# fdb/frequensea

Hardware: AMD Instinct MI355X
Metric: fft_frames_per_sec_n8192 (higher is better)
Workload: dtype f32

## Files before the change

### frequensea_amd/csrc/fsea_fft_core.h

```cpp
#pragma once

#include <hip/hip_runtime.h>
#include <stddef.h>
#include <stdint.h>

#include <fsea_pk_asm.h>
#include "fsea_opt.h"
#ifdef FSEA_TUNE
#include <fsea_pk_asm_tune.h>
#endif

namespace fsea {

constexpr int ilog2c(int n) {
    int l = 0;
    while ((1 << l) < n) ++l;
    return l;
}

constexpr int bitrev_c(int i, int bits) {
    int r = 0;
    for (int b = 0; b < bits; ++b) {
        if (i & (1 << b)) r |= 1 << (bits - 1 - b);
    }
    return r;
}

template <int P>
__host__ __device__ constexpr int lds_pad(int idx) {
    return idx + ((idx / P) << 1);
}

__host__ __device__ constexpr float cos64q(int i) {
    constexpr float t[17] = {1.000000000e+00f, 9.951847267e-01f, 9.807852804e-01f,
                             9.569403357e-01f, 9.238795325e-01f, 8.819212643e-01f,
                             8.314696123e-01f, 7.730104534e-01f, 7.071067812e-01f,
                             6.343932842e-01f, 5.555702330e-01f, 4.713967368e-01f,
                             3.826834324e-01f, 2.902846773e-01f, 1.950903220e-01f,
                             9.801714033e-02f, 0.0f};
    return t[i];
}
__host__ __device__ constexpr float cos64(int m) {
    m &= 63;
    if (m <= 16) return cos64q(m);
    if (m <= 32) return -cos64q(32 - m);
    if (m <= 48) return -cos64q(m - 32);
    return cos64q(64 - m);
}
__host__ __device__ constexpr float sin64(int m) { return cos64((m - 16) & 63); }

__device__ __forceinline__ cf cf_swap(cf b) { return __builtin_shufflevector(b, b, 1, 0); }
__device__ __forceinline__ cf cf_fma(cf a, cf b, cf c) { return __builtin_elementwise_fma(a, b, c); }

template <int L, int K>
__device__ __forceinline__ void bfly_const(cf &a, cf &b) {
    if constexpr (K == 0) {
        const cf t = b;
        b = a - t;
        a = a + t;
    } else if constexpr (4 * K == L) {
        const cf t = b;
        b = pk_add_pi(a, t);
        a = pk_add_mi(a, t);
    } else {
        constexpr int m = K * (64 / L);
        constexpr float wr = cos64(m), wi = -sin64(m);
        cf plus = cf_fma(b, cf{wr, wr}, a);
        plus = cf_fma(cf_swap(b), cf{-wi, wi}, plus);
        b = cf_fma(a, cf{2.0f, 2.0f}, -plus);
        a = plus;
    }
}

template <int R, int HALF, int BASE = 0, int K = 0>
__device__ __forceinline__ void dft_const_level(cf *y) {
    if constexpr (BASE < R) {
        bfly_const<2 * HALF, K>(y[BASE + K], y[BASE + K + HALF]);
        if constexpr (K + 1 < HALF) dft_const_level<R, HALF, BASE, K + 1>(y);
        else dft_const_level<R, HALF, BASE + 2 * HALF, 0>(y);
    }
}
template <int R, int HALF>
__device__ __forceinline__ void dft_const_levels(cf *y) {
    if constexpr (HALF < R) {
        dft_const_level<R, HALF>(y);
// ... 12 lines not shown
    dft_const_levels<R, 1>(y);
#pragma unroll
    for (int i = 0; i < R; ++i) x[i * S] = y[i];
}

template <int R, int S, int E0, int I = 0>
__device__ __forceinline__ void dft_win_level(const cf *x, const cf *wv, cf *y) {
    if constexpr (I < R / 2) {
        constexpr int BITS = ilog2c(R), EA = E0 + I * S, EB = E0 + (I + R / 2) * S;
        const cf a = x[I * S], b = x[(I + R / 2) * S];
        cf t;
        if constexpr (EB & 1) t = pk_scale_hi(b, wv[EB / 2]);
        else t = pk_scale_lo(b, wv[EB / 2]);
        if constexpr (EA & 1) {
            y[bitrev_c(I, BITS)] = pk_wfma_hi(a, wv[EA / 2], t);
            y[bitrev_c(I + R / 2, BITS)] = pk_wfms_hi(a, wv[EA / 2], t);
        } else {
            y[bitrev_c(I, BITS)] = pk_wfma_lo(a, wv[EA / 2], t);
            y[bitrev_c(I + R / 2, BITS)] = pk_wfms_lo(a, wv[EA / 2], t);
        }
        dft_win_level<R, S, E0, I + 1>(x, wv, y);
    }
}
template <int R, int S, int E0>
__device__ __forceinline__ void dft_regs_win(cf *x, const cf *wv) {
    static_assert(R >= 2 && R <= 64 && (R & (R - 1)) == 0, "radix must be 2..64");
    cf y[R];
    dft_win_level<R, S, E0>(x, wv, y);
    dft_const_levels<R, 2>(y);
#pragma unroll
    for (int i = 0; i < R; ++i) x[i * S] = y[i];
}

template <int R, int S, int TS>
__device__ __forceinline__ void dft_regs_tw(cf *x, const cf *tw, float sc0) {
    static_assert(R >= 4 && R <= 64 && (R & (R - 1)) == 0, "radix must be 4..64");
    constexpr int BITS = ilog2c(R);
    cf y[R];
#pragma unroll
    for (int i = 0; i < R / 2; ++i) {
        cf a = x[i * S];
        if (i == 0) {
            if (sc0 != 1.0f) a = a * cf{sc0, sc0};
        } else {
            a = pk_cmul(a, tw[(i - 1) * TS]);
        }
        const cf plus = pk_cmul_add(x[(i + R / 2) * S], tw[(i + R / 2 - 1) * TS], a);
        y[bitrev_c(i, BITS)] = plus;
        y[bitrev_c(i + R / 2, BITS)] = cf_fma(a, cf{2.0f, 2.0f}, -plus);
    }
    dft_const_levels<R, 2>(y);
#pragma unroll
    for (int i = 0; i < R; ++i) x[i * S] = y[i];
}

template <int R, int HALF, int TS, int DROP = 0>
__device__ __forceinline__ void dft_def_level(cf *y, const cf *tw) {
    if constexpr (HALF < R) {
        constexpr int OFF = HALF / 2, DISTINCT = HALF >= 2 ? HALF / 2 : 1;
#pragma unroll
        for (int base = 0; base < R; base += 2 * HALF) {
#pragma unroll
            for (int k = 0; k < DISTINCT; ++k) {
                cf &a = y[base + k], &b = y[base + k + HALF];
                const cf plus = pk_cmul_add(b, tw[(OFF + k) * TS], a);
                if constexpr (HALF <= DROP) b = a;
                else b = cf_fma(a, cf{2.0f, 2.0f}, -plus);
                a = plus;
            }
            if constexpr (HALF >= 2) {
#pragma unroll
                for (int k = 0; k < DISTINCT; ++k) {
                    cf &a = y[base + DISTINCT + k], &b = y[base + DISTINCT + k + HALF];
                    const cf plus = pk_cmul_add_mi(b, tw[(OFF + k) * TS], a);
                    if constexpr (HALF <= DROP) b = a;
                    else b = cf_fma(a, cf{2.0f, 2.0f}, -plus);
                    a = plus;
                }
            }
        }
        dft_def_level<R, 2 * HALF, TS, DROP>(y, tw);
    }
}

template <int R, int S, int TS, int DROP = 0>
__device__ __forceinline__ void dft_regs_def(cf *x, const cf *tw) {
    static_assert(R >= 4 && R <= 64 && (R & (R - 1)) == 0, "radix must be 4..64");
    constexpr int BITS = ilog2c(R);
    cf y[R];
#pragma unroll
    for (int i = 0; i < R; ++i) y[bitrev_c(i, BITS)] = x[i * S];
    dft_def_level<R, 1, TS, DROP>(y, tw);
#pragma unroll
    for (int i = 0; i < R; ++i) x[i * S] = y[i];
}

enum : int {
    MODE_MAG = 0,
    MODE_DB10_U8 = 1,
    MODE_DB5_U8_DCFIX = 2,
    MODE_COMPLEX = 3,
    MODE_MAG_NODC = 4,
    MODE_DB_F32 = 5
};
enum : int { IN_U8 = 0, IN_F32 = 1, IN_U8_ROT = 2 };

#ifndef FSEA_DEFAULT_OPT
#define FSEA_DEFAULT_OPT 0
#endif
#ifndef FSEA_STATIC_CONTIG
#define FSEA_STATIC_CONTIG 0
#endif
#ifndef FSEA_TRACE
#define FSEA_TRACE 0
#endif

template <int N_, int T_, int FPW_, int WPE_, int NP_, int R0_, int R1_, int R2_ = 1, int R3_ = 1,
          bool TWL_ = true, bool TWR_ = true, int ABL_ = 0, int OPT_ = FSEA_DEFAULT_OPT>
struct FftCfg {
    static constexpr int OPT = OPT_;
    static constexpr int ABL = ABL_;
    static constexpr int N = N_, T = T_, FPW = FPW_, NP = NP_;
    static constexpr int WPE = WPE_;
    static constexpr int P = N_ / T_;
    static constexpr int WG = T_ * FPW_;
// ... 40 lines not shown
    const float *win = nullptr;
    const cf *win_dc = nullptr;
    uint32_t win_offset = 0;
};

template <int C>
__device__ __forceinline__ void ld_c(const cf *p, cf *dst) {
    if constexpr (C == 1) {
        dst[0] = *p;
    } else {
#pragma unroll
        for (int c = 0; c < C; c += 2) {
            const cf2 q = *reinterpret_cast<const cf2 *>(p + c);
            dst[c] = cf{q[0], q[1]};
            dst[c + 1] = cf{q[2], q[3]};
        }
    }
}

template <int C>
__device__ __forceinline__ void st_c(cf *p, const cf *src) {
    if constexpr (C == 1) {
        *p = src[0];
    } else {
#pragma unroll
        for (int c = 0; c < C; c += 2) {
            *reinterpret_cast<cf2 *>(p + c) = cf2{src[c][0], src[c][1], src[c + 1][0], src[c + 1][1]};
        }
    }
}

typedef __amdgpu_buffer_rsrc_t rsrc_t;

__device__ __forceinline__ rsrc_t buffer_window(const void *base, size_t off, size_t total) {
    const size_t rem = total > off ? total - off : 0;
    char *p = const_cast<char *>(static_cast<const char *>(base)) + (rem ? off : 0);
    return __builtin_amdgcn_make_buffer_rsrc(p, 0, rem > 0xffffffffull ? 0xffffffffu : (uint32_t)rem, 0x00020000);
}

typedef uint32_t u32x2 __attribute__((vector_size(8)));
typedef uint32_t u32x4 __attribute__((vector_size(16)));

__device__ __forceinline__ uint32_t f2u(float x) { return __builtin_bit_cast(uint32_t, x); }
__device__ __forceinline__ float u2f(uint32_t x) { return __builtin_bit_cast(float, x); }

#ifndef FSEA_STORE_GUARD
#define FSEA_STORE_GUARD 1
#endif
__device__ __forceinline__ void store_data_guard() {
#if !defined(__AMDGCN__)
#elif FSEA_STORE_GUARD == 1
    __builtin_amdgcn_sched_barrier(0);
    asm volatile("s_nop 7\n\ts_nop 7");
    __builtin_amdgcn_sched_barrier(0);
#elif FSEA_STORE_GUARD >= 10
    __builtin_amdgcn_sched_barrier(0);
    asm volatile("s_nop %0" ::"n"(FSEA_STORE_GUARD - 10));
    __builtin_amdgcn_sched_barrier(0);
#endif
}

template <int AUX>
__device__ __forceinline__ void bst128(rsrc_t rs, uint32_t voff, uint32_t soff, u32x4 data) {
#if FSEA_STORE_GUARD == 2
    __builtin_amdgcn_raw_buffer_store_b64(u32x2{data[0], data[1]}, rs, voff, soff, AUX);
    __builtin_amdgcn_raw_buffer_store_b64(u32x2{data[2], data[3]}, rs, voff + 8, soff, AUX);
#else
    __builtin_amdgcn_raw_buffer_store_b128(data, rs, voff, soff, AUX);
    store_data_guard();
#endif
// ... 99 lines not shown
    double s, c;
    sincospi(2.0 * turns, &s, &c);
    return cf{(float)c, (float)s};
}
__device__ __forceinline__ cf turn_phasor_f32(double turns) {
    turns -= floor(turns);
    float s, c;
    sincospif(2.0f * (float)turns, &s, &c);
    return cf{c, s};
}

template <class Cfg, int IN, int MODE_T = -1, bool ROT = false, bool RUNS = false, int WIN = 0>
struct FftKernel {
    static_assert(!ROT || IN == IN_U8, "the fused frequency shift is a u8-input path");
    static_assert(WIN == 0 || (Cfg::TWR && (Cfg::OPT & opt::TUNE_ONLY) == 0 && Cfg::P >= 8),
                  "the windowed kernels: V1 schedule, register-resident last-pass twiddles");
    static_assert(WIN == 0 || !RUNS || (IN == IN_U8 && !ROT), "windowed half-overlap runs: the plain u8 kernel only");
    static constexpr bool WIN_DC = WIN != 0 && IN == IN_U8;
    static constexpr bool LATE_LOAD = WIN != 0 && IN == IN_F32;
    static constexpr bool DC_IN_REGS = WIN_DC && ((Cfg::OPT & opt::WIN_DC_REGS) != 0 ||
                                                  ((Cfg::OPT & opt::WIN_DC_REGS_MAG) != 0 && MODE_T == MODE_MAG && !ROT));
    static_assert(!RUNS || (IN == IN_U8 && !ROT && Cfg::FPW == 1 && (Cfg::R(0) % 2) == 0), "half-overlap runs: u8 input, one frame per workgroup");
    static constexpr int N = Cfg::N, T = Cfg::T, P = Cfg::P, NP = Cfg::NP, FPW = Cfg::FPW;
    static constexpr int LAST = NP - 1;
    static constexpr int R0 = Cfg::R(0), C0 = Cfg::C(0);
    static constexpr int RL = Cfg::R(LAST), CL = Cfg::C(LAST), NsL = Cfg::Ns(LAST);
    static constexpr bool ONE_WAVE = (Cfg::WG <= 64) || (T <= 64 && (64 % T) == 0);
    static constexpr float SC = (IN == IN_U8) ? (1.0f / 256.0f) : 1.0f;
    static constexpr bool PRESCALED = Cfg::TWR && (IN == IN_U8);
    using Raw = RawRow<IN, C0>;
    static constexpr bool BATCH_READS = (Cfg::OPT & opt::BATCH_READS) != 0;
    static constexpr bool TW_HOIST = (Cfg::OPT & opt::TW_HOIST) != 0;
    static constexpr bool TW_FUSE = (Cfg::OPT & opt::TW_FUSE) != 0 && (Cfg::ABL & abl::NO_FLOPS) == 0;
    static constexpr int ST_AUX = (Cfg::OPT & opt::ST_NT) ? 2 : 0;
    template <int ELEM_BYTES>
    static constexpr int st_aux() { return (T * CL * ELEM_BYTES >= 128 && CL * ELEM_BYTES <= 16) ? ST_AUX : (ST_AUX & ~2); }
    static constexpr int LD_AUX = (Cfg::OPT & opt::LD_NT) ? 2 : 0;
    static constexpr bool DEFER = (Cfg::OPT & opt::DEFER) != 0 && NP == 3;
    static constexpr bool PX_PACK = (Cfg::OPT & opt::PX_PACK) != 0;
    static constexpr bool PX_BIAS = (Cfg::OPT & opt::PX_BIAS) != 0;
    static constexpr bool LANE_ROT = (Cfg::OPT & opt::LANE_ROT) != 0;
    static constexpr bool LANE_ROT_LAST = (Cfg::OPT & opt::LANE_ROT_LAST) != 0;
    template <int I>
    static __device__ __forceinline__ int pass_lane(int t) {
        constexpr bool ON = (I == LAST) ? LANE_ROT_LAST : LANE_ROT;
        if constexpr (ON && Cfg::C(I) == 2 && P == 32 && (T % 16) == 0) {
            const int blk = t >> 4;
            return (blk << 4) | ((t - blk) & 15);
        } else if constexpr (ON && Cfg::C(I) == 1 && P == 16 && T == 256) {
            const int blk = t >> 4;
            const int logical = (blk >> 1) | ((blk & 1) << 3);
            return (logical << 4) | (t & 15);
        } else {
            return t;
        }
    }

    static __device__ __forceinline__ void after_reads() {
        if constexpr (BATCH_READS) __builtin_amdgcn_sched_barrier(0);
    }

    static __device__ __forceinline__ void frame_sync() {
        if constexpr (Cfg::ABL & abl::NO_LDS) {
            return;
        } else if constexpr (ONE_WAVE) {
            __builtin_amdgcn_fence(__ATOMIC_RELEASE, "wavefront");
// ... 105 lines not shown
                for (int r = 0; r < R; ++r) lds[Cfg::pad(j0 + r * Ns)] = v[r * C + c];
            }
        }
    }

    template <int I>
    static __device__ __forceinline__ void lds_read(const cf *lds, cf *v, int t) {
        constexpr int R = Cfg::R(I), C = Cfg::C(I);
        constexpr int STRIDE = N / R;
        if constexpr (Cfg::ABL & abl::NO_LDS) {
            return;
        } else if constexpr (STRIDE % P == 0) {
            const cf *base = lds + Cfg::pad(C * t);
#pragma unroll
            for (int r = 0; r < R; ++r) ld_c<C>(base + r * (STRIDE + 2 * (STRIDE / P)), v + r * C);
        } else {
#pragma unroll
            for (int r = 0; r < R; ++r) ld_c<C>(lds + Cfg::pad(C * t + r * STRIDE), v + r * C);
        }
    }

    template <int I>
    static __device__ __forceinline__ void middle_pass(cf *lds, const cf *lds_all, cf *v, const FftArgs &a, int t0,
                                                       const cf *tw_res = nullptr) {
        if constexpr (I < LAST) {
            constexpr int R = Cfg::R(I), C = Cfg::C(I);
            const int t = pass_lane<I>(t0);
            const cf *tw = Cfg::TWL ? (lds_all + Cfg::lds_tw_off(I)) : a.tw[I];
            if constexpr (DEFER) {
                lds_read<I>(lds, v, t);
                after_reads();
                frame_sync();
#pragma unroll
                for (int c = 0; c < C; ++c) dft_regs_def<R, C, 1, (Cfg::ABL & abl::DROP_32_OPS) ? 2 : ((Cfg::ABL & abl::DROP_16_OPS) ? 1 : 0)>(v + c, tw_res + c * (R / 2));
            } else if constexpr (TW_HOIST && (Cfg::Ns(I) % C == 0)) {
                constexpr int Ns = Cfg::Ns(I);
                cf w[(R - 1) * C];
                const int k0 = (C * t) % Ns;
#pragma unroll
                for (int r = 1; r < R; ++r) ld_c<C>(tw + (r - 1) * Ns + k0, w + (r - 1) * C);
                lds_read<I>(lds, v, t);
                after_reads();
                frame_sync();
                if constexpr (TW_FUSE) {
#pragma unroll
                    for (int c = 0; c < C; ++c) dft_regs_tw<R, C, C>(v + c, w + c, 1.0f);
                } else {
#pragma unroll
                    for (int r = 1; r < R; ++r) {
#pragma unroll
                        for (int c = 0; c < C; ++c) v[r * C + c] = pk_cmul(v[r * C + c], w[(r - 1) * C + c]);
                    }
                }
            } else {
                lds_read<I>(lds, v, t);
                after_reads();
                frame_sync();
                apply_twiddles<I>(v, tw, t);
            }
            if constexpr (!DEFER && !(TW_FUSE && TW_HOIST && (Cfg::Ns(I) % C == 0))) {
#pragma unroll
                for (int c = 0; c < C; ++c) dft_regs<R, C, (Cfg::ABL & abl::NO_FLOPS) != 0>(v + c);
            }
            lds_write<I>(lds, v, t);
            frame_sync();
            middle_pass<I + 1>(lds, lds_all, v, a, t0, tw_res);
        }
    }

    static __device__ __forceinline__ uint32_t elem_bytes(int mode) {
        return (mode == MODE_DB10_U8 || mode == MODE_DB5_U8_DCFIX) ? 1u : (mode == MODE_COMPLEX ? 8u : 4u);
    }

    static __device__ __forceinline__ float bin_power(const cf *v, int r, int c) {
        const cf z = v[r * CL + c];
        return __builtin_fmaf(z[0], z[0], z[1] * z[1]);
    }

    static __device__ __forceinline__ void epilogue(int mode, rsrc_t out, uint32_t lane_elem, cf *v, int t) {
        constexpr float SE = PRESCALED ? 1.0f : SC;
        constexpr float SE2 = SE * SE;
        const bool patched = (mode == MODE_MAG) || (mode == MODE_DB5_U8_DCFIX);
        if (WIN == 0 && IN == IN_U8 && !patched && t == 0) {
            const float dc = (PRESCALED ? 0.5f : 128.0f) * (float)N;
            v[(RL / 2) * CL] += cf{dc, dc};
        }
        if (mode == MODE_COMPLEX) {
            const uint32_t voff = lane_elem * 8u;
#pragma unroll
            for (int r = 0; r < RL; ++r) {
                cf z[CL];
#pragma unroll
                for (int c = 0; c < CL; ++c) z[c] = v[r * CL + c] * cf{SE, SE};
                bst<CL, st_aux<8>()>(out, voff, (uint32_t)(r * NsL) * 8u, z);
            }
        } else if (mode == MODE_DB10_U8 || mode == MODE_DB5_U8_DCFIX) {
            const float kdb = (mode == MODE_DB10_U8 ? 100.0f : 50.0f) * 0.30102999566398120f;
            const uint32_t voff = lane_elem;
#pragma unroll
            for (int r = 0; r < RL; ++r) {
                const uint32_t soff = (uint32_t)(r * NsL);
                uint8_t px[CL];
                [[maybe_unused]] uint32_t pxw[(CL + 3) / 4] = {};
#pragma unroll
                for (int c = 0; c < CL; ++c) {
                    float p = bin_power(v, r, c);
                    if constexpr (!PRESCALED && IN == IN_U8) p *= SE2;
                    if constexpr (PX_PACK) {
                        float d;
                        if constexpr (PX_BIAS) d = __builtin_fmaf(kdb, __builtin_amdgcn_logf(p), -0.49999997f);
                        else d = trunc_f32(kdb * __builtin_amdgcn_logf(p));
                        if constexpr (Cfg::ABL & abl::NO_EPILOGUE_MATH) d = kdb * p;
                        pxw[c / 4] = cvt_pk_u8(d, (uint32_t)(c & 3), pxw[c / 4]);
                    } else {
                        float d = kdb * __builtin_amdgcn_logf(p);
                        if constexpr (Cfg::ABL & abl::NO_EPILOGUE_MATH) d = kdb * p;
                        int q = (int)d;
                        q = q < 0 ? 0 : (q > 255 ? 255 : q);
                        px[c] = (uint8_t)q;
                    }
                }
                if constexpr (PX_PACK) {
#pragma unroll
                    for (int c = 0; c < CL; ++c) px[c] = (uint8_t)(pxw[c / 4] >> (8 * (c & 3)));
                }
                if constexpr (Cfg::ABL & abl::NO_STORES) {
                    if (px[0] == 255 && px[CL - 1] == 254 && v[0][0] == -1.0f) bst<CL>(out, voff, soff, px);
                } else if (patched && r == RL / 2 && t == 0) {
#pragma unroll
                    for (int c = 1; c < CL; ++c) bst<1>(out, voff + c, soff, px + c);
                } else if constexpr (PX_PACK) {
                    if constexpr (CL == 1) __builtin_amdgcn_raw_buffer_store_b8((uint8_t)pxw[0], out, voff, soff, st_aux<1>());
                    else if constexpr (CL == 2) __builtin_amdgcn_raw_buffer_store_b16((uint16_t)pxw[0], out, voff, soff, st_aux<1>());
                    else {
#pragma unroll
                        for (int c = 0; c < CL; c += 4) __builtin_amdgcn_raw_buffer_store_b32(pxw[c / 4], out, voff + c, soff, st_aux<1>());
                    }
                } else {
                    bst<CL, st_aux<1>()>(out, voff, soff, px);
                }
                if (patched && r == RL / 2 - 1 && t == T - 1) bst<1>(out, voff + CL, soff, px + (CL - 1));
            }
        } else if (mode == MODE_DB_F32) {
            f32_rows<true>(patched, out, lane_elem, v, t);
        } else {
            f32_rows<false>(patched, out, lane_elem, v, t);
        }
    }

    template <bool LOG>
    static __device__ __forceinline__ void f32_rows(bool patched, rsrc_t out, uint32_t lane_elem, cf *v, int t) {
        constexpr float SE = PRESCALED ? 1.0f : SC;
        constexpr float SE2 = SE * SE;
        const uint32_t voff = lane_elem * 4u;
#pragma unroll
        for (int r = 0; r < RL; ++r) {
            const uint32_t soff = (uint32_t)(r * NsL) * 4u;
            float m[CL];
#pragma unroll
            for (int c = 0; c < CL; ++c) {
                float p = bin_power(v, r, c);
                if constexpr (!PRESCALED && IN == IN_U8) p *= SE2;
                if constexpr (LOG) {
                    m[c] = (10.0f * 0.30102999566398120f) * __builtin_amdgcn_logf(p + 1.0e-20f);
                } else if constexpr (Cfg::ABL & abl::NO_EPILOGUE_MATH) {
                    m[c] = v[r * CL + c][0];
                } else {
                    m[c] = __builtin_amdgcn_sqrtf(p);
                }
            }
            if constexpr (Cfg::ABL & abl::NO_STORES) {
                if (m[0] == -1.0f) bst<CL>(out, voff, soff, m);
            } else if (patched && r == RL / 2 && t == 0) {
#pragma unroll
                for (int c = 1; c < CL; ++c) bst<1>(out, voff + 4 * c, soff, m + c);
                if constexpr (CL >= 4) store_data_guard();
            } else {
                bst<CL, st_aux<4>()>(out, voff, soff, m);
            }
            if (patched && r == RL / 2 - 1 && t == T - 1) bst<1>(out, voff + 4 * CL, soff, m + (CL - 1));
        }
    }

    static constexpr bool DYNAMIC = !ONE_WAVE;
    static constexpr unsigned POOLS = 8;
    static constexpr unsigned NO_UNIT = 0xffffffffu;

    struct Pools {
        unsigned n_units, grid;
        __device__ __forceinline__ unsigned start(unsigned q) const { return (unsigned)((size_t)n_units * q / POOLS); }
        __device__ __forceinline__ unsigned homed(unsigned q) const { return (grid + POOLS - 1 - q) / POOLS; }
        __device__ __forceinline__ unsigned unit(unsigned q, unsigned t) const {
            const unsigned long long idx = (unsigned long long)start(q) + homed(q) + t;
            return idx < start(q + 1) ? (unsigned)idx : NO_UNIT;
        }
    };

#ifdef FSEA_TUNE
    static constexpr bool V2 = (Cfg::OPT & opt::V2) != 0, W64 = (Cfg::OPT & opt::W64) != 0;
#else
    static constexpr bool V2 = false, W64 = false;
    static_assert((Cfg::OPT & opt::TUNE_ONLY) == 0 && Cfg::ABL == 0, "tuning-only option or ablation in a product build");
#endif
    static constexpr int counters_used() { return W64 ? 0 : (V2 ? 2 : (DYNAMIC ? 1 : 0)); }

    static constexpr int WPAIRS = WIN ? P / 2 : 1;
    static constexpr int DC_OFF = (Cfg::LDS_ALLOC + 1) & ~1;
    static constexpr int LDS_CF = (WIN_DC && !DC_IN_REGS) ? DC_OFF + 2 * NsL : Cfg::LDS_ALLOC;
    static constexpr int DC_REGS = (2 * NsL + Cfg::WG - 1) / Cfg::WG;
    static_assert(WIN == 0 || (Cfg::TWL || Cfg::TWR), "the DC table rides on the table block's barrier");
    static __device__ __forceinline__ void load_window(rsrc_t rs, int t, cf *wv) {
        const uint32_t voff = (uint32_t)t * 16u;
#pragma unroll
// ... 42 lines not shown

    static __device__ __forceinline__ void run_v1(const FftArgs &a, cf *lds_all) {
        const int tid = threadIdx.x;
        const int slot = (FPW == 1) ? 0 : tid / T;
        const int t = (FPW == 1) ? tid : tid % T;
        cf *lds = lds_all + slot * Cfg::LDS_FRAME;
        unsigned *tk = reinterpret_cast<unsigned *>(lds_all + Cfg::LDS_TOTAL);

        const unsigned b = blockIdx.x;
        const bool issuer = (tid == 0);
        const size_t n_units = RUNS ? (a.n_frames + a.run_len - 1) / a.run_len : (a.n_frames + FPW - 1) / FPW;
        Pools pools;
        pools.n_units = (unsigned)n_units;
        pools.grid = gridDim.x;
        unsigned cur = b % POOLS;

        if ((FSEA_TRACE != 0) && a.trace != nullptr && tid == 0) {
            const unsigned hw_id = read_hw_id(), xcc_id = read_xcc_id();
            a.trace[32 * b + 0] = wall_clock64();
            a.trace[32 * b + 2] = __builtin_readcyclecounter();
            a.trace[32 * b + 4] = hw_id;
            a.trace[32 * b + 5] = xcc_id;
        }

        const int mode = (MODE_T >= 0) ? MODE_T : a.mode;
        const uint32_t xormask = (MODE_T >= 0) ? 0u : a.xormask;
        const uint32_t esz = elem_bytes(mode);
        const size_t total_in = (size_t)IN_BPS * ((a.n_frames - 1) * a.hop + (size_t)N);
        const bool tiled = a.tile_rows != 0;
        const size_t total_out = (size_t)esz * (tiled ? a.out_span : a.n_frames * (size_t)N);
        const uint32_t in_voff = (uint32_t)IN_BPS * ((uint32_t)slot * (uint32_t)a.hop + (uint32_t)(C0 * t));
        const int tl = pass_lane<LAST>(t);
        const uint32_t out_elem = (uint32_t)slot * (tiled ? a.pitch_row : (uint32_t)N) + (uint32_t)(CL * tl);
        auto row_elem = [&](size_t f) -> size_t {
            if (!tiled) return f * (size_t)N;
            const uint32_t k = (uint32_t)f / a.tile_rows, y = (uint32_t)f - k * a.tile_rows;
            return (size_t)y * a.pitch_row + (size_t)k * a.pitch_tile;
        };

        size_t u = b;
#if FSEA_STATIC_CONTIG
        [[maybe_unused]] const size_t contig_per = (n_units + gridDim.x - 1) / gridDim.x;
        [[maybe_unused]] size_t contig_end = n_units;
        if constexpr (!RUNS) {
            u = (size_t)b * contig_per;
            contig_end = u + contig_per < n_units ? u + contig_per : n_units;
            if (u >= n_units) u = n_units;
        }
#endif
        unsigned tick_next = 0;
        const bool dyn = !RUNS && DYNAMIC && a.dynamic_units != 0;
        [[maybe_unused]] size_t fcur = RUNS ? (size_t)b * a.run_len : 0;
        [[maybe_unused]] unsigned jpos = 0;
        if (dyn) {
            u = (size_t)pools.start(cur) + b / POOLS;
            if (u >= pools.start(cur + 1)) u = n_units;
        }
        constexpr int TAB_COPY = (Cfg::TWL || Cfg::TWR) ? Cfg::TAB_SMALL : 0;
        constexpr int TAB_REGS = (TAB_COPY + Cfg::WG - 1) / Cfg::WG;
        cf tabv[TAB_REGS > 0 ? TAB_REGS : 1];
#pragma unroll
        for (int i = 0; i < TAB_REGS; ++i) {
            const int e = tid + i * Cfg::WG;
            tabv[i] = a.tw_small[e < TAB_COPY ? e : TAB_COPY - 1];
        }
        constexpr int R1 = Cfg::R(1), C1 = Cfg::C(1), Ns1 = Cfg::Ns(1);
        cf tw1[DEFER ? C1 * (R1 / 2) : 1];
        if constexpr (DEFER) {
            const int t1 = pass_lane<1>(t);
#pragma unroll
            for (int c = 0; c < C1; ++c) ld_c<R1 / 2>(a.tw_def + ((C1 * t1 + c) % Ns1) * (R1 / 2), tw1 + c * (R1 / 2));
        }
        [[maybe_unused]] const rsrc_t win_rs = buffer_window(WIN ? a.win : nullptr, 0, WIN ? (size_t)N * 4u : 0);
        cf wv[WPAIRS];
        cf dcv[(WIN_DC && !DC_IN_REGS) ? DC_REGS : 1];
        cf dcr[DC_IN_REGS ? 2 * CL : 1];
        if constexpr (DC_IN_REGS) {
#pragma unroll
            for (int c = 0; c < CL; ++c) {
                dcr[c] = a.win_dc[CL * tl + c];
                dcr[CL + c] = a.win_dc[NsL + CL * tl + c];
            }
        }
        if constexpr (WIN != 0) load_window(win_rs, t, wv);
        if constexpr (WIN_DC && !DC_IN_REGS) {
#pragma unroll
            for (int i = 0; i < DC_REGS; ++i) {
                const int e = tid + i * Cfg::WG;
                dcv[i] = a.win_dc[e < 2 * NsL ? e : 2 * NsL - 1];
            }
        }
        if (dyn) {
            if (issuer) tick_next = atomicAdd(a.ctr + 32 * cur, 1u);
        }
        Raw raw[R0];
        load_raw(buffer_window(a.in, (size_t)IN_BPS * (RUNS ? fcur : u * FPW) * a.hop, u < n_units ? total_in : 0), in_voff, raw);
        balance_vmcnt();

        if constexpr (TAB_COPY > 0) {
#pragma unroll
            for (int i = 0; i < TAB_REGS; ++i) {
                const int e = tid + i * Cfg::WG;
                lds_all[FPW * Cfg::LDS_FRAME + (e < TAB_COPY ? e : TAB_COPY - 1)] = tabv[i];
            }
            if constexpr (WIN_DC && !DC_IN_REGS) {
#pragma unroll
                for (int i = 0; i < DC_REGS; ++i) {
                    const int e = tid + i * Cfg::WG;
                    lds_all[DC_OFF + (e < 2 * NsL ? e : 2 * NsL - 1)] = dcv[i];
                }
            }
            if ((FSEA_TRACE != 0) && a.trace != nullptr && tid == 0) a.trace[32 * b + 28] = wall_clock64();
            __syncthreads();
            if ((FSEA_TRACE != 0) && a.trace != nullptr && tid == 0) a.trace[32 * b + 29] = wall_clock64();
        }
        cf twl[Cfg::TWR ? (RL - 1) * CL : 1];
        if constexpr (Cfg::TWR) {
            const cf *hi = lds_all + Cfg::LDS_HI, *lo = lds_all + Cfg::LDS_LO;
            auto root = [&](unsigned m) -> cf { return pk_cmul(hi[m >> 6], lo[m & 63u]); };
            constexpr int RB = RL >= 16 ? 8 : (RL >= 4 ? 2 : RL);
            constexpr int RA = RL / RB;
#pragma unroll
            for (int c = 0; c < CL; ++c) {
                const unsigned k = (unsigned)(CL * tl + c);
                cf wb[RB], wa[RA];
#pragma unroll
                for (int bb = 1; bb < RB; ++bb) wb[bb] = root((unsigned)bb * k);
#pragma unroll
                for (int aa = 1; aa < RA; ++aa) wa[aa] = root((unsigned)(RB * aa) * k);
#pragma unroll
                for (int r = 1; r < RL; ++r) {
                    const int aa = r / RB, bb = r % RB;
                    cf w = aa == 0 ? wb[bb] : (bb == 0 ? wa[aa] : pk_cmul(wa[aa], wb[bb]));
                    if constexpr (PRESCALED) w = w * cf{SC, SC};
                    twl[(r - 1) * CL + c] = w;
                }
            }
        }

        cf ebase[ROT ? C0 : 1];
        if constexpr (ROT) {
#pragma unroll
            for (int c = 0; c < C0; ++c) {
                const unsigned n0 = (unsigned)(C0 * t + c);
                const cf e = turn_phasor_f64(a.rot_delta * (double)n0);
                ebase[c] = (WIN == 0 && (n0 & 1u)) ? -e : e;
            }
        }

        unsigned par = 0;
        if (dyn && u >= n_units) {
            if (issuer) {
                unsigned nu = pools.unit(cur, tick_next);
                for (unsigned k = 1; nu == NO_UNIT && k < POOLS; ++k) {
                    const unsigned q = (cur + k) % POOLS;
                    nu = pools.unit(q, atomicAdd(a.ctr + 32 * q, 1u));
                    if (nu != NO_UNIT) cur = q;
                }
                tk[0] = nu;
                tick_next = atomicAdd(a.ctr + 32 * cur, 1u);
            }
            __syncthreads();
            const unsigned nu = __builtin_amdgcn_readfirstlane(tk[0]);
            __syncthreads();
            u = (nu == NO_UNIT) ? n_units : (size_t)nu;
            load_raw(buffer_window(a.in, (size_t)IN_BPS * (u * FPW) * a.hop, u < n_units ? total_in : 0), in_voff, raw);
            balance_vmcnt();
        }

        unsigned iter = 0;
        if ((FSEA_TRACE != 0) && a.trace != nullptr && tid == 0) a.trace[32 * b + 6] = wall_clock64();
        while (u < n_units) {
            if (dyn && issuer) {
                unsigned nu = pools.unit(cur, tick_next);
                for (unsigned k = 1; nu == NO_UNIT && k < POOLS; ++k) {
                    const unsigned q = (cur + k) % POOLS;
                    nu = pools.unit(q, atomicAdd(a.ctr + 32 * q, 1u));
                    if (nu != NO_UNIT) cur = q;
                }
                tk[par] = nu;
                tick_next = atomicAdd(a.ctr + 32 * cur, 1u);
            }

            cf v[P];
            if constexpr (ROT) {
                const size_t first = (u * FPW + (size_t)slot) * a.hop;
                const cf ef = turn_phasor_f32(a.rot_phase0 + a.rot_delta * (double)first);
                cf fr[C0];
#pragma unroll
                for (int c = 0; c < C0; ++c) fr[c] = pk_cmul(ebase[c], ef);
#pragma unroll
                for (int r = 0; r < R0; ++r) {
                    convert_row<IN, C0, false>(raw[r], a.xormask, C0 * t, v + r * C0);
                    const cf wr = a.rot_row[r];
#pragma unroll
                    for (int c = 0; c < C0; ++c) {
                        v[r * C0 + c] = pk_cmul(v[r * C0 + c] + cf{128.0f, 128.0f}, pk_cmul_uniform(fr[c], wr));
                        if constexpr (WIN != 0) {
                            if (a.win_offset != 0) v[r * C0 + c] += cf{128.0f, 128.0f};
                        }
                    }
                }
            } else if constexpr (WIN != 0 && IN == IN_F32) {
#pragma unroll
                for (int r = 0; r < R0; ++r) convert_row<IN, C0, false>(raw[r], 0u, C0 * t, v + r * C0);
// ... 5 lines not shown
                for (int r = 0; r < R0; ++r) convert_row<IN, C0>(raw[r], xormask, C0 * t, v + r * C0);
            }
            if ((FSEA_TRACE != 0) && a.trace != nullptr && tid == 0 && iter == 0) {
                asm volatile("" ::"v"(v[0]));
                a.trace[32 * b + 30] = wall_clock64();
            }
            if constexpr (WIN != 0) {
                pass0_windowed(v, wv);
            } else {
#pragma unroll
                for (int c = 0; c < C0; ++c) dft_regs<R0, C0, (Cfg::ABL & abl::NO_FLOPS) != 0>(v + c);
            }
            lds_write<0>(lds, v, t);
            frame_sync();
            if ((FSEA_TRACE != 0) && a.trace != nullptr && tid == 0 && iter == 0) a.trace[32 * b + 7] = wall_clock64();
            size_t un = u + gridDim.x;
#if FSEA_STATIC_CONTIG
            if constexpr (!RUNS) un = u + 1 < contig_end ? u + 1 : n_units;
#endif
            [[maybe_unused]] size_t fnext = 0;
            [[maybe_unused]] bool same_run = false;
            if constexpr (RUNS) {
                same_run = (jpos + 1 < a.run_len) && (fcur + 1 < a.n_frames);
                un = same_run ? u : u + gridDim.x;
                fnext = same_run ? fcur + 1 : un * (size_t)a.run_len;
            }
            if (dyn) {
                if constexpr (Cfg::ABL & abl::NO_LDS) __syncthreads();
                const unsigned nu = __builtin_amdgcn_readfirstlane(tk[par]);
                par ^= 1u;
                un = (nu == NO_UNIT) ? n_units : (size_t)nu;
            }
            if constexpr (RUNS) {
                const rsrc_t rs = buffer_window(a.in, (size_t)IN_BPS * fnext * a.hop, un < n_units ? total_in : 0);
                if (same_run) {
#pragma unroll
                    for (int r = 0; r < R0 / 2; ++r) raw[r] = raw[r + R0 / 2];
                    load_raw_rows<R0 / 2, R0>(rs, in_voff, raw);
                } else {
                    load_raw(rs, in_voff, raw);
                }
            } else if constexpr ((Cfg::ABL & abl::NO_LOADS) == 0 && !LATE_LOAD) {
                load_raw(buffer_window(a.in, (size_t)IN_BPS * (un * FPW) * a.hop, un < n_units ? total_in : 0), in_voff, raw);
            }
            middle_pass<1>(lds, lds_all, v, a, t, tw1);

            lds_read<LAST>(lds, v, tl);
            after_reads();
            frame_sync();
            if constexpr (Cfg::TWR && TW_FUSE) {
#pragma unroll
                for (int c = 0; c < CL; ++c) dft_regs_tw<RL, CL, CL>(v + c, twl + c, PRESCALED ? SC : 1.0f);
            } else if constexpr (Cfg::TWR) {
                if constexpr (PRESCALED) {
#pragma unroll
                    for (int c = 0; c < CL; ++c) v[c] = v[c] * cf{SC, SC};
                }
#pragma unroll
                for (int r = 1; r < RL; ++r) {
#pragma unroll
                    for (int c = 0; c < CL; ++c) {
                        if constexpr (Cfg::ABL & abl::NO_FLOPS) v[r * CL + c] += twl[(r - 1) * CL + c];
                        else v[r * CL + c] = pk_cmul(v[r * CL + c], twl[(r - 1) * CL + c]);
                    }
                }
            } else {
                apply_twiddles<LAST>(v, a.tw[LAST], tl);
            }
            if constexpr (!(Cfg::TWR && TW_FUSE)) {
#pragma unroll
                for (int c = 0; c < CL; ++c) dft_regs<RL, CL, (Cfg::ABL & abl::NO_FLOPS) != 0>(v + c);
            }
            if constexpr (DC_IN_REGS) {
#pragma unroll
                for (int c = 0; c < CL; ++c) {
                    v[(RL / 2 - 1) * CL + c] += dcr[c];
                    v[(RL / 2) * CL + c] += dcr[CL + c];
                }
            }
            if constexpr (WIN_DC && !DC_IN_REGS) {
                constexpr int CB = CL >= 2 ? 2 : 1;
#pragma unroll
                for (int c = 0; c < CL; c += CB) {
                    cf dc_lo[CB], dc_hi[CB];
                    ld_c<CB>(lds_all + DC_OFF + CL * tl + c, dc_lo);
                    ld_c<CB>(lds_all + DC_OFF + NsL + CL * tl + c, dc_hi);
#pragma unroll
                    for (int j = 0; j < CB; ++j) {
                        v[(RL / 2 - 1) * CL + c + j] += dc_lo[j];
                        v[(RL / 2) * CL + c + j] += dc_hi[j];
                    }
                }
            }
            if constexpr (WIN != 0) {
                if constexpr (WIN == 1) {
                    load_window(win_rs, t, wv);
                    __builtin_amdgcn_sched_barrier(0);
                }
            }
            epilogue(mode, buffer_window(a.out, (size_t)esz * row_elem(RUNS ? fcur : u * FPW), total_out), out_elem, v, tl);
            if constexpr (LATE_LOAD) {
                load_raw(buffer_window(a.in, (size_t)IN_BPS * (un * FPW) * a.hop, un < n_units ? total_in : 0), in_voff, raw);
            }
            u = un;
            if constexpr (RUNS) {
                fcur = fnext;
                jpos = same_run ? jpos + 1 : 0;
            }
            if ((FSEA_TRACE != 0) && a.trace != nullptr && tid == 0 && iter < 24) a.trace[32 * b + 8 + iter] = wall_clock64();
            ++iter;
        }

        if (dyn && issuer) {
            __builtin_amdgcn_s_waitcnt(0);
            const unsigned finished = atomicAdd(a.ctr + 32 * POOLS, 1u);
            if (finished == gridDim.x - 1) {
#pragma unroll
                for (unsigned q = 0; q <= POOLS; ++q) a.ctr[32 * q] = 0;
            }
        }
        if ((FSEA_TRACE != 0) && a.trace != nullptr && tid == 0) {
            a.trace[32 * b + 1] = wall_clock64();
            a.trace[32 * b + 3] = __builtin_readcyclecounter();
        }
    }
};

}
```

Measured before the change: 86.33 million.

## Fuse twiddle butterflies into packed-FMA asm and force scalar unit-window math

Adds inline-asm packed FMA sequences that compute the twiddled butterfly (plus and minus outputs) in three v_pk_fma instructions, used in the register DFT passes for the plain u8 input kernel. It also moves the buffer-window and unit-bound computations onto scalar registers via readfirstlane so the 64-bit comparisons are not done per lane. Lane-flag checks in the epilogue are forced into VGPRs to steer codegen. The aim is fewer VALU instructions and less vector register pressure, at the risk of the hand-written asm defeating compiler scheduling or carrying op_sel mistakes.

```diff
diff --git a/frequensea_amd/csrc/fsea_fft_core.h b/frequensea_amd/csrc/fsea_fft_core.h
--- a/frequensea_amd/csrc/fsea_fft_core.h
+++ b/frequensea_amd/csrc/fsea_fft_core.h
@@ -6,6 +6,7 @@
 
 #include <fsea_pk_asm.h>
 #include "fsea_opt.h"
+#include "fsea_unit_window.h"
 #ifdef FSEA_TUNE
 #include <fsea_pk_asm_tune.h>
 #endif
@@ -51,6 +52,10 @@
 
 __device__ __forceinline__ cf cf_swap(cf b) { return __builtin_shufflevector(b, b, 1, 0); }
 __device__ __forceinline__ cf cf_fma(cf a, cf b, cf c) { return __builtin_elementwise_fma(a, b, c); }
+
+}
+#include "fsea_pk_fused.h"
+namespace fsea {
 
 template <int L, int K>
 __device__ __forceinline__ void bfly_const(cf &a, cf &b) {
@@ -129,7 +134,7 @@
     for (int i = 0; i < R; ++i) x[i * S] = y[i];
 }
 
-template <int R, int S, int TS>
+template <int R, int S, int TS, bool FUSED = false>
 __device__ __forceinline__ void dft_regs_tw(cf *x, const cf *tw, float sc0) {
     static_assert(R >= 4 && R <= 64 && (R & (R - 1)) == 0, "radix must be 4..64");
     constexpr int BITS = ilog2c(R);
@@ -139,19 +144,27 @@
         cf a = x[i * S];
         if (i == 0) {
             if (sc0 != 1.0f) a = a * cf{sc0, sc0};
+        } else if constexpr (FUSED) {
+            a = pk_cmul_fused(a, tw[(i - 1) * TS]);
         } else {
             a = pk_cmul(a, tw[(i - 1) * TS]);
         }
-        const cf plus = pk_cmul_add(x[(i + R / 2) * S], tw[(i + R / 2 - 1) * TS], a);
-        y[bitrev_c(i, BITS)] = plus;
-        y[bitrev_c(i + R / 2, BITS)] = cf_fma(a, cf{2.0f, 2.0f}, -plus);
+        if constexpr (FUSED) {
+            cf b = x[(i + R / 2) * S];
+            y[bitrev_c(i, BITS)] = pk_bfly_cmul(a, b, tw[(i + R / 2 - 1) * TS]);
+            y[bitrev_c(i + R / 2, BITS)] = b;
+        } else {
+            const cf plus = pk_cmul_add(x[(i + R / 2) * S], tw[(i + R / 2 - 1) * TS], a);
+            y[bitrev_c(i, BITS)] = plus;
+            y[bitrev_c(i + R / 2, BITS)] = cf_fma(a, cf{2.0f, 2.0f}, -plus);
+        }
     }
     dft_const_levels<R, 2>(y);
 #pragma unroll
     for (int i = 0; i < R; ++i) x[i * S] = y[i];
 }
 
-template <int R, int HALF, int TS, int DROP = 0>
+template <int R, int HALF, int TS, int DROP = 0, bool FUSED = false>
 __device__ __forceinline__ void dft_def_level(cf *y, const cf *tw) {
     if constexpr (HALF < R) {
         constexpr int OFF = HALF / 2, DISTINCT = HALF >= 2 ? HALF / 2 : 1;
@@ -160,34 +173,42 @@
 #pragma unroll
             for (int k = 0; k < DISTINCT; ++k) {
                 cf &a = y[base + k], &b = y[base + k + HALF];
-                const cf plus = pk_cmul_add(b, tw[(OFF + k) * TS], a);
-                if constexpr (HALF <= DROP) b = a;
-                else b = cf_fma(a, cf{2.0f, 2.0f}, -plus);
-                a = plus;
-            }
-            if constexpr (HALF >= 2) {
-#pragma unroll
-                for (int k = 0; k < DISTINCT; ++k) {
-                    cf &a = y[base + DISTINCT + k], &b = y[base + DISTINCT + k + HALF];
-                    const cf plus = pk_cmul_add_mi(b, tw[(OFF + k) * TS], a);
+                if constexpr (FUSED && HALF > DROP) {
+                    a = pk_bfly_cmul(a, b, tw[(OFF + k) * TS]);
+                } else {
+                    const cf plus = pk_cmul_add(b, tw[(OFF + k) * TS], a);
                     if constexpr (HALF <= DROP) b = a;
                     else b = cf_fma(a, cf{2.0f, 2.0f}, -plus);
                     a = plus;
                 }
             }
-        }
-        dft_def_level<R, 2 * HALF, TS, DROP>(y, tw);
-    }
-}
-
-template <int R, int S, int TS, int DROP = 0>
+            if constexpr (HALF >= 2) {
+#pragma unroll
+                for (int k = 0; k < DISTINCT; ++k) {
+                    cf &a = y[base + DISTINCT + k], &b = y[base + DISTINCT + k + HALF];
+                    if constexpr (FUSED && HALF > DROP) {
+                        a = pk_bfly_cmul_mi(a, b, tw[(OFF + k) * TS]);
+                    } else {
+                        const cf plus = pk_cmul_add_mi(b, tw[(OFF + k) * TS], a);
+                        if constexpr (HALF <= DROP) b = a;
+                        else b = cf_fma(a, cf{2.0f, 2.0f}, -plus);
+                        a = plus;
+                    }
+                }
+            }
+        }
+        dft_def_level<R, 2 * HALF, TS, DROP, FUSED>(y, tw);
+    }
+}
+
+template <int R, int S, int TS, int DROP = 0, bool FUSED = false>
 __device__ __forceinline__ void dft_regs_def(cf *x, const cf *tw) {
     static_assert(R >= 4 && R <= 64 && (R & (R - 1)) == 0, "radix must be 4..64");
     constexpr int BITS = ilog2c(R);
     cf y[R];
 #pragma unroll
     for (int i = 0; i < R; ++i) y[bitrev_c(i, BITS)] = x[i * S];
-    dft_def_level<R, 1, TS, DROP>(y, tw);
+    dft_def_level<R, 1, TS, DROP, FUSED>(y, tw);
 #pragma unroll
     for (int i = 0; i < R; ++i) x[i * S] = y[i];
 }
@@ -294,10 +315,17 @@
 
 typedef __amdgpu_buffer_rsrc_t rsrc_t;
 
+template <bool SCALAR = false>
 __device__ __forceinline__ rsrc_t buffer_window(const void *base, size_t off, size_t total) {
-    const size_t rem = total > off ? total - off : 0;
-    char *p = const_cast<char *>(static_cast<const char *>(base)) + (rem ? off : 0);
-    return __builtin_amdgcn_make_buffer_rsrc(p, 0, rem > 0xffffffffull ? 0xffffffffu : (uint32_t)rem, 0x00020000);
+    if constexpr (SCALAR) {
+        const ByteWindow w = byte_window(off, total);
+        char *p = const_cast<char *>(static_cast<const char *>(base)) + w.base_off;
+        return __builtin_amdgcn_make_buffer_rsrc(p, 0, w.num_records, 0x00020000);
+    } else {
+        const size_t rem = total > off ? total - off : 0;
+        char *p = const_cast<char *>(static_cast<const char *>(base)) + (rem ? off : 0);
+        return __builtin_amdgcn_make_buffer_rsrc(p, 0, rem > 0xffffffffull ? 0xffffffffu : (uint32_t)rem, 0x00020000);
+    }
 }
 
 typedef uint32_t u32x2 __attribute__((vector_size(8)));
@@ -463,6 +491,8 @@
     static constexpr bool BATCH_READS = (Cfg::OPT & opt::BATCH_READS) != 0;
     static constexpr bool TW_HOIST = (Cfg::OPT & opt::TW_HOIST) != 0;
     static constexpr bool TW_FUSE = (Cfg::OPT & opt::TW_FUSE) != 0 && (Cfg::ABL & abl::NO_FLOPS) == 0;
+    static constexpr bool PK_FUSED = WIN == 0 && IN == IN_U8 && !ROT;
+    static constexpr bool SCALAR_UNITS = PK_FUSED;
     static constexpr int ST_AUX = (Cfg::OPT & opt::ST_NT) ? 2 : 0;
     template <int ELEM_BYTES>
     static constexpr int st_aux() { return (T * CL * ELEM_BYTES >= 128 && CL * ELEM_BYTES <= 16) ? ST_AUX : (ST_AUX & ~2); }
@@ -634,7 +664,7 @@
                 after_reads();
                 frame_sync();
 #pragma unroll
-                for (int c = 0; c < C; ++c) dft_regs_def<R, C, 1, (Cfg::ABL & abl::DROP_32_OPS) ? 2 : ((Cfg::ABL & abl::DROP_16_OPS) ? 1 : 0)>(v + c, tw_res + c * (R / 2));
+                for (int c = 0; c < C; ++c) dft_regs_def<R, C, 1, (Cfg::ABL & abl::DROP_32_OPS) ? 2 : ((Cfg::ABL & abl::DROP_16_OPS) ? 1 : 0), PK_FUSED>(v + c, tw_res + c * (R / 2));
             } else if constexpr (TW_HOIST && (Cfg::Ns(I) % C == 0)) {
                 constexpr int Ns = Cfg::Ns(I);
                 cf w[(R - 1) * C];
@@ -646,7 +676,7 @@
                 frame_sync();
                 if constexpr (TW_FUSE) {
 #pragma unroll
-                    for (int c = 0; c < C; ++c) dft_regs_tw<R, C, C>(v + c, w + c, 1.0f);
+                    for (int c = 0; c < C; ++c) dft_regs_tw<R, C, C, PK_FUSED>(v + c, w + c, 1.0f);
                 } else {
 #pragma unroll
                     for (int r = 1; r < R; ++r) {
@@ -677,6 +707,17 @@
     static __device__ __forceinline__ float bin_power(const cf *v, int r, int c) {
         const cf z = v[r * CL + c];
         return __builtin_fmaf(z[0], z[0], z[1] * z[1]);
+    }
+
+    static __device__ __forceinline__ bool lane_flag(bool f) {
+#if defined(__AMDGCN__)
+        if constexpr (PK_FUSED && MODE_T >= 0 && CL <= 2) {
+            uint32_t x = f ? 1u : 0u;
+            asm("" : "+v"(x));
+            return x != 0;
+        }
+#endif
+        return f;
     }
 
     static __device__ __forceinline__ void epilogue(int mode, rsrc_t out, uint32_t lane_elem, cf *v, int t) {
@@ -699,6 +740,7 @@
         } else if (mode == MODE_DB10_U8 || mode == MODE_DB5_U8_DCFIX) {
             const float kdb = (mode == MODE_DB10_U8 ? 100.0f : 50.0f) * 0.30102999566398120f;
             const uint32_t voff = lane_elem;
+            const bool first_lane = lane_flag(t == 0), last_lane = lane_flag(t == T - 1);
 #pragma unroll
             for (int r = 0; r < RL; ++r) {
                 const uint32_t soff = (uint32_t)(r * NsL);
@@ -728,7 +770,7 @@
                 }
                 if constexpr (Cfg::ABL & abl::NO_STORES) {
                     if (px[0] == 255 && px[CL - 1] == 254 && v[0][0] == -1.0f) bst<CL>(out, voff, soff, px);
-                } else if (patched && r == RL / 2 && t == 0) {
+                } else if (patched && r == RL / 2 && first_lane) {
 #pragma unroll
                     for (int c = 1; c < CL; ++c) bst<1>(out, voff + c, soff, px + c);
                 } else if constexpr (PX_PACK) {
@@ -741,7 +783,7 @@
                 } else {
                     bst<CL, st_aux<1>()>(out, voff, soff, px);
                 }
-                if (patched && r == RL / 2 - 1 && t == T - 1) bst<1>(out, voff + CL, soff, px + (CL - 1));
+                if (patched && r == RL / 2 - 1 && last_lane) bst<1>(out, voff + CL, soff, px + (CL - 1));
             }
         } else if (mode == MODE_DB_F32) {
             f32_rows<true>(patched, out, lane_elem, v, t);
@@ -755,6 +797,7 @@
         constexpr float SE = PRESCALED ? 1.0f : SC;
         constexpr float SE2 = SE * SE;
         const uint32_t voff = lane_elem * 4u;
+        const bool first_lane = lane_flag(t == 0), last_lane = lane_flag(t == T - 1);
 #pragma unroll
         for (int r = 0; r < RL; ++r) {
             const uint32_t soff = (uint32_t)(r * NsL) * 4u;
@@ -773,14 +816,14 @@
             }
             if constexpr (Cfg::ABL & abl::NO_STORES) {
                 if (m[0] == -1.0f) bst<CL>(out, voff, soff, m);
-            } else if (patched && r == RL / 2 && t == 0) {
+            } else if (patched && r == RL / 2 && first_lane) {
 #pragma unroll
                 for (int c = 1; c < CL; ++c) bst<1>(out, voff + 4 * c, soff, m + c);
                 if constexpr (CL >= 4) store_data_guard();
             } else {
                 bst<CL, st_aux<4>()>(out, voff, soff, m);
             }
-            if (patched && r == RL / 2 - 1 && t == T - 1) bst<1>(out, voff + 4 * CL, soff, m + (CL - 1));
+            if (patched && r == RL / 2 - 1 && last_lane) bst<1>(out, voff + 4 * CL, soff, m + (CL - 1));
         }
     }
 
@@ -889,11 +932,9 @@
         const uint32_t in_voff = (uint32_t)IN_BPS * ((uint32_t)slot * (uint32_t)a.hop + (uint32_t)(C0 * t));
         const int tl = pass_lane<LAST>(t);
         const uint32_t out_elem = (uint32_t)slot * (tiled ? a.pitch_row : (uint32_t)N) + (uint32_t)(CL * tl);
-        auto row_elem = [&](size_t f) -> size_t {
-            if (!tiled) return f * (size_t)N;
-            const uint32_t k = (uint32_t)f / a.tile_rows, y = (uint32_t)f - k * a.tile_rows;
-            return (size_t)y * a.pitch_row + (size_t)k * a.pitch_tile;
-        };
+        auto row_elem = [&](size_t f) -> size_t { return row_element(f, (uint32_t)N, a.tile_rows, a.pitch_row, a.pitch_tile); };
+        auto has_unit = [&](size_t unit) -> bool { return SCALAR_UNITS ? lt_u63(unit, n_units) : unit < n_units; };
+        auto window = [&](const void *base, size_t off, size_t total) -> rsrc_t { return buffer_window<SCALAR_UNITS>(base, off, total); };
 
         size_t u = b;
 #if FSEA_STATIC_CONTIG
@@ -951,7 +992,7 @@
             if (issuer) tick_next = atomicAdd(a.ctr + 32 * cur, 1u);
         }
         Raw raw[R0];
-        load_raw(buffer_window(a.in, (size_t)IN_BPS * (RUNS ? fcur : u * FPW) * a.hop, u < n_units ? total_in : 0), in_voff, raw);
+        load_raw(window(a.in, (size_t)IN_BPS * (RUNS ? fcur : u * FPW) * a.hop, has_unit(u) ? total_in : 0), in_voff, raw);
         balance_vmcnt();
 
         if constexpr (TAB_COPY > 0) {
@@ -1006,7 +1047,7 @@
         }
 
         unsigned par = 0;
-        if (dyn && u >= n_units) {
+        if (dyn && !has_unit(u)) {
             if (issuer) {
                 unsigned nu = pools.unit(cur, tick_next);
                 for (unsigned k = 1; nu == NO_UNIT && k < POOLS; ++k) {
@@ -1021,13 +1062,13 @@
             const unsigned nu = __builtin_amdgcn_readfirstlane(tk[0]);
             __syncthreads();
             u = (nu == NO_UNIT) ? n_units : (size_t)nu;
-            load_raw(buffer_window(a.in, (size_t)IN_BPS * (u * FPW) * a.hop, u < n_units ? total_in : 0), in_voff, raw);
+            load_raw(window(a.in, (size_t)IN_BPS * (u * FPW) * a.hop, has_unit(u) ? total_in : 0), in_voff, raw);
             balance_vmcnt();
         }
 
         unsigned iter = 0;
         if ((FSEA_TRACE != 0) && a.trace != nullptr && tid == 0) a.trace[32 * b + 6] = wall_clock64();
-        while (u < n_units) {
+        while (has_unit(u)) {
             if (dyn && issuer) {
                 unsigned nu = pools.unit(cur, tick_next);
                 for (unsigned k = 1; nu == NO_UNIT && k < POOLS; ++k) {
@@ -1099,7 +1140,7 @@
                 un = (nu == NO_UNIT) ? n_units : (size_t)nu;
             }
             if constexpr (RUNS) {
-                const rsrc_t rs = buffer_window(a.in, (size_t)IN_BPS * fnext * a.hop, un < n_units ? total_in : 0);
+                const rsrc_t rs = window(a.in, (size_t)IN_BPS * fnext * a.hop, has_unit(un) ? total_in : 0);
                 if (same_run) {
 #pragma unroll
                     for (int r = 0; r < R0 / 2; ++r) raw[r] = raw[r + R0 / 2];
@@ -1108,7 +1149,7 @@
                     load_raw(rs, in_voff, raw);
                 }
             } else if constexpr ((Cfg::ABL & abl::NO_LOADS) == 0 && !LATE_LOAD) {
-                load_raw(buffer_window(a.in, (size_t)IN_BPS * (un * FPW) * a.hop, un < n_units ? total_in : 0), in_voff, raw);
+                load_raw(window(a.in, (size_t)IN_BPS * (un * FPW) * a.hop, has_unit(un) ? total_in : 0), in_voff, raw);
             }
             middle_pass<1>(lds, lds_all, v, a, t, tw1);
 
@@ -1117,7 +1158,7 @@
             frame_sync();
             if constexpr (Cfg::TWR && TW_FUSE) {
 #pragma unroll
-                for (int c = 0; c < CL; ++c) dft_regs_tw<RL, CL, CL>(v + c, twl + c, PRESCALED ? SC : 1.0f);
+                for (int c = 0; c < CL; ++c) dft_regs_tw<RL, CL, CL, PK_FUSED>(v + c, twl + c, PRESCALED ? SC : 1.0f);
             } else if constexpr (Cfg::TWR) {
                 if constexpr (PRESCALED) {
 #pragma unroll
@@ -1165,9 +1206,9 @@
                     __builtin_amdgcn_sched_barrier(0);
                 }
             }
-            epilogue(mode, buffer_window(a.out, (size_t)esz * row_elem(RUNS ? fcur : u * FPW), total_out), out_elem, v, tl);
+            epilogue(mode, window(a.out, (size_t)esz * row_elem(RUNS ? fcur : u * FPW), total_out), out_elem, v, tl);
             if constexpr (LATE_LOAD) {
-                load_raw(buffer_window(a.in, (size_t)IN_BPS * (un * FPW) * a.hop, un < n_units ? total_in : 0), in_voff, raw);
+                load_raw(window(a.in, (size_t)IN_BPS * (un * FPW) * a.hop, has_unit(un) ? total_in : 0), in_voff, raw);
             }
             u = un;
             if constexpr (RUNS) {
diff --git a/frequensea_amd/csrc/fsea_pk_fused.h b/frequensea_amd/csrc/fsea_pk_fused.h
--- /dev/null
+++ b/frequensea_amd/csrc/fsea_pk_fused.h
@@ -0,0 +1,45 @@
+#pragma once
+
+namespace fsea {
+
+__device__ __forceinline__ cf pk_cmul_fused(cf a, cf w) {
+#if defined(__AMDGCN__)
+    cf t;
+    asm("v_pk_mul_f32 %0, %1, %2 op_sel_hi:[1,0]\n\t"
+        "v_pk_fma_f32 %0, %1, %2, %0 op_sel:[1,1,0] op_sel_hi:[0,1,1] neg_lo:[0,1,0]" : "=&v"(t) : "v"(a), "v"(w));
+    return t;
+#else
+    return pk_cmul(a, w);
+#endif
+}
+
+__device__ __forceinline__ cf pk_bfly_cmul(cf a, cf &b, cf w) {
+#if defined(__AMDGCN__)
+    cf plus;
+    asm("v_pk_fma_f32 %0, %1, %2, %3 op_sel_hi:[1,0,1]\n\t"
+        "v_pk_fma_f32 %0, %1, %2, %0 op_sel:[1,1,0] op_sel_hi:[0,1,1] neg_lo:[0,1,0]\n\t"
+        "v_pk_fma_f32 %1, %3, 2.0, %0 op_sel_hi:[1,0,1] neg_lo:[0,0,1] neg_hi:[0,0,1]"
+        : "=&v"(plus), "+v"(b) : "v"(w), "v"(a));
+    return plus;
+#else
+    const cf plus = pk_cmul_add(b, w, a);
+    b = cf_fma(a, cf{2.0f, 2.0f}, -plus);
+    return plus;
+#endif
+}
+__device__ __forceinline__ cf pk_bfly_cmul_mi(cf a, cf &b, cf w) {
+#if defined(__AMDGCN__)
+    cf plus;
+    asm("v_pk_fma_f32 %0, %1, %2, %3 op_sel:[0,1,0] op_sel_hi:[1,1,1]\n\t"
+        "v_pk_fma_f32 %0, %1, %2, %0 op_sel:[1,0,0] op_sel_hi:[0,0,1] neg_hi:[0,1,0]\n\t"
+        "v_pk_fma_f32 %1, %3, 2.0, %0 op_sel_hi:[1,0,1] neg_lo:[0,0,1] neg_hi:[0,0,1]"
+        : "=&v"(plus), "+v"(b) : "v"(w), "v"(a));
+    return plus;
+#else
+    const cf plus = pk_cmul_add_mi(b, w, a);
+    b = cf_fma(a, cf{2.0f, 2.0f}, -plus);
+    return plus;
+#endif
+}
+
+}
diff --git a/frequensea_amd/csrc/fsea_unit_window.h b/frequensea_amd/csrc/fsea_unit_window.h
--- /dev/null
+++ b/frequensea_amd/csrc/fsea_unit_window.h
@@ -0,0 +1,59 @@
+#pragma once
+
+#include <stddef.h>
+#include <stdint.h>
+
+#ifndef __HIPCC__
+#ifndef __host__
+#define __host__
+#endif
+#ifndef __device__
+#define __device__
+#endif
+#endif
+
+namespace fsea {
+
+__host__ __device__ inline uint32_t opaque_scalar(uint32_t x) {
+#if defined(__AMDGCN__)
+    return __builtin_amdgcn_readfirstlane(x);
+#else
+#if defined(__GNUC__)
+    asm("" : "+r"(x));
+#endif
+    return x;
+#endif
+}
+
+__host__ __device__ inline bool lt_u63(uint64_t a, uint64_t b) { return (int32_t)opaque_scalar((uint32_t)((a - b) >> 32)) < 0; }
+
+struct ByteWindow {
+    uint64_t base_off;
+    uint32_t num_records;
+};
+__host__ __device__ inline ByteWindow byte_window(uint64_t off, uint64_t total) {
+    const uint64_t d = total - off;
+    const uint32_t hi = opaque_scalar((uint32_t)(d >> 32));
+    const bool none = (int32_t)hi < 0;
+    const uint32_t rem_hi = none ? 0u : hi, rem_lo = none ? 0u : (uint32_t)d;
+    ByteWindow w;
+    w.base_off = (rem_hi | rem_lo) != 0 ? off : 0;
+    w.num_records = rem_hi != 0 ? 0xffffffffu : rem_lo;
+    return w;
+}
+
+__host__ __device__ inline uint64_t row_element(uint64_t f, uint32_t n, uint32_t tile_rows, uint32_t pitch_row, uint32_t pitch_tile) {
+    if (tile_rows == 0) return f * (uint64_t)n;
+    const uint32_t k = (uint32_t)f / tile_rows, y = (uint32_t)f - k * tile_rows;
+    return (uint64_t)y * pitch_row + (uint64_t)k * pitch_tile;
+}
+
+__host__ __device__ inline ByteWindow unit_input_window(uint64_t u, uint64_t n_units, uint32_t fpw, uint64_t hop, uint32_t bps, uint64_t total_in) {
+    return byte_window((uint64_t)bps * (u * fpw) * hop, lt_u63(u, n_units) ? total_in : 0);
+}
+__host__ __device__ inline ByteWindow unit_output_window(uint64_t f, uint32_t n, uint32_t esz, uint32_t tile_rows, uint32_t pitch_row,
+                                                         uint32_t pitch_tile, uint64_t total_out) {
+    return byte_window((uint64_t)esz * row_element(f, n, tile_rows, pitch_row, pitch_tile), total_out);
+}
+
+}
```

Result: no change. 87.15 million (median of 6 runs) (+1.0%).
